# fukangl/SMG-multimodal-grasping

Measured on AMD Instinct MI355X. Metric: affordance fwd+bwd passes/sec (16-rot 224^2 RGB-D), higher is better.
Workload: dtype f32; 1 GPU; 16 rot x 224^2 (S=640): fwd + Huber + bwd + Adam per GPU per step; reinforcement_net style 0; 17 trunk passes; fp32; leg=headline, rotations=16, input_size=640, parallelism=dp1

## Files before the change

### smg-multimodal-grasping_amd/csrc/backward.hip

```cpp
#include "engine.h"

static void pick_chunk(const Plane& pl, int n_planes, int tiles_per_chunk, int& chunk, int& cps, int target = 768) {
    const int want = (target + tiles_per_chunk - 1) / tiles_per_chunk;
    cps = (want + n_planes - 1) / n_planes;
    if (cps < 1) cps = 1;
    chunk = ((pl.HW + cps - 1) / cps + 63) / 64 * 64;
    cps = (pl.HW + chunk - 1) / chunk;
}

int do_backward(smg_engine* e, const smg_net* net, const float* dq, hipStream_t st, int phases) {
    if (!e->have_fwd) return fail(-22, "smg_backward without a preceding smg_forward");
    if (!net->grads) return fail(-22, "net.grads is NULL");
    if (phases == 2 && !e->bw_phase0_done)
        return fail(-22, "smg_backward_phase(1) must follow smg_backward_phase(0) of the same forward");
    if ((phases & 1) && e->bw_phase0_done)
        return fail(-22, "smg_backward / smg_backward_phase(0) while the second half of a two-phase backward is still due (run phase 1 or a new forward)");
    const Layout& L = *e->L;
    const TrunkRef& T = L.trunk[e->f_trunk];
    const HeadRef& Hd = L.head[e->f_head];
    const int NS = e->f_streams, NP = e->f_pairs;
    const float* P = net->params;
    float* Gr = net->grads;
    const Plane p4 = e->p_blk[3];
    const bool ph_a = phases & 1, ph_b = phases & 2;
    if (ph_a) {
        for (int r = 0; r < kStatRep; ++r) HIP_OK(hipMemsetAsync(e->bstat + (size_t)r * kStatRepStride, 0, 2 * e->bstat_span * sizeof(double), st));
    }
    const bool split16 = e->prec == 0 && kSplitOp == 3;
    if (ph_a && split16) HIP_OK(hipMemsetAsync(e->gamax, 0, (size_t)e->gamax_words * sizeof(unsigned), st));
    const hipStream_t s2 = (e->prof || e->serialize) ? st : e->side;
    auto fork = [&](hipEvent_t ev) -> int {
        HIP_OK(hipEventRecord(ev, st));
        HIP_OK(hipStreamWaitEvent(s2, ev, 0));
        return 0;
    };
    const bool gs_materialised = split16 || NS > 4;
    auto gs_on_side = [&](const Plane& pl) { return split16 && !e->generic3x3 && pl.HW <= 1600 && NS <= 4; };
    auto launch_gs_apply = [&](int b, int i, hipStream_t cs, float* GSb) {
        const Plane pl = e->p_blk[b];
        const int Ct = kBlockCtot[b];
        const DenseLayerRef& d = T.layers[b][i];
        BnBwdApplyArgs a{};
        a.g = e->G[b]; a.ldg = Ct; a.gcoff = d.cin; a.x = e->X[b]; a.ldx = Ct; a.xcoff = d.cin; a.pl = pl; a.C = kGrowth;
        a.xsum = fsum(e, e->st_X[b]); a.xsq = fsq(e, e->st_X[b]); a.xstride = Ct; a.xtab = stat_table(e, e->sx_tab[b], e->max_streams, Ct);
        a.s1 = b1(e, e->st_X[b]); a.s2 = b2(e, e->st_X[b]); a.sstride = Ct; a.scoff = d.cin; a.gamma = nullptr; a.eps = kEps;
        a.out = GSb; a.ldo = kGrowth; a.amax = split16 ? gamax_of(e, b, i, 0) : nullptr;
        PREC_DISPATCH(e, launch_kernel(e, bn_bwd_apply_kernel<PREC>, dim3((pl.HWp + bn_apply_rows(PREC) - 1) / bn_apply_rows(PREC), NS), dim3(256), 0, cs,
                                       K_OTHER, 0, ESZ(e) * NS * pl.HW * 3 * kGrowth, false, a));
    };

    if (ph_a) {
    {
        ValueBwdArgs a;
// ... 194 lines not shown
            float* bt = el(e, e->Bt, e->bt_off[b][i]);
            const LayerBuf lb = buf_of(b, i);
            float* GSb = lb.GS;
            float* D2b = lb.D2;
            static_assert(kRing % 3 == 0 && kRing > 3, "the sparse ring wait covers three slots at a time");
            if (lb.ring >= kRing && lb.ring % 3 == 0) HIP_OK(hipStreamWaitEvent(st, e->ev_side[(lb.ring + 2) % kRing], 0));
            GradSrc gsrc{};
            gsrc.g = el(e, e->G[b], d.cin); gsrc.ldg = Ct; gsrc.x = el(e, e->X[b], d.cin); gsrc.ldx = Ct;
            gsrc.xsum = fsum(e, e->st_X[b]) + d.cin; gsrc.xsq = fsq(e, e->st_X[b]) + d.cin;
            gsrc.s1 = b1(e, e->st_X[b]) + d.cin; gsrc.s2 = b2(e, e->st_X[b]) + d.cin; gsrc.sstride = Ct; gsrc.eps = kEps;
            if (e->generic3x3 || (gs_materialised && !gs_on_side(pl))) {
                launch_gs_apply(b, i, st, GSb);
                if (gs_materialised) { gsrc = GradSrc{}; gsrc.g = GSb; gsrc.ldg = kGrowth; gsrc.amax = gamax_of(e, b, i, 0); }
            }
            if (!e->generic3x3) {
                Halo3x3DgradArgs a;
                a.g = gsrc; a.pl = pl; a.C = kBottleneck;
                a.mbuf = bt;
                a.dst = split16 ? e->DY2 : D2b; a.o1 = b1(e, e->st_Bt[b][i]); a.o2 = b2(e, e->st_Bt[b][i]); a.ostride = kBottleneck;
                a.wu = e->packed_u + e->pk_hd[b][i]; a.bt = bn_table(e, e->sb_tab[b][i], e->max_streams, 0, kBottleneck, P + d.n2.w, P + d.n2.b);
                const double flops = 2.0 * NS * pl.HW * 9 * kBottleneck * kGrowth;
                const double bytes = ESZ(e) * NS * pl.HW * (kGrowth + 2 * kBottleneck);
                if (halo_tile(pl, NS) == 16) {
                    a.tiles_x = (pl.W + 15) / 16; a.cg_per_wg = kBottleneck / 32;
                    if (pl.H % 16 || pl.W % 16) {
                        PREC_DISPATCH(e, launch_kernel(e, conv3x3_halo_dgrad_kernel<16, PREC, true>, dim3(((pl.H + 15) / 16) * a.tiles_x, NS), dim3(256),
                                                       HaloDgradSGeo<16, PREC>::smem_bytes(kBottleneck), st, K_D3, flops, bytes, true, a));
                    } else {
                        PREC_DISPATCH(e, launch_kernel(e, conv3x3_halo_dgrad_kernel<16, PREC>, dim3((pl.H / 16) * a.tiles_x, NS), dim3(256),
                                                       HaloDgradSGeo<16, PREC>::smem_bytes(kBottleneck), st, K_D3, flops, bytes, true, a));
                    }
                } else {
                    a.tiles_x = (pl.W + 7) / 8; a.cg_per_wg = 1;
                    PREC_DISPATCH(e, launch_kernel(e, conv3x3_halo_dgrad_kernel<8, PREC>, dim3(((pl.H + 7) / 8) * a.tiles_x, NS, kBottleneck / 64), dim3(256),
                                                   HaloDgradSGeo<8, PREC>::smem_bytes(kBottleneck), st, K_D3, flops, bytes, true, a));
                }
            } else {
                auto run = [&](auto tag) {
                    using Cfg = decltype(tag);
                    BwdDataP<Cfg, true, E_STORE, false> p{};
                    p.gbuf = GSb; p.ldg = kGrowth; p.gcoff = 0; p.xbuf = nullptr; p.pa = pl; p.KA = kGrowth;
                    p.wp = e->packed_u + e->pk_g3d[b][i]; p.K8tot = 9 * kGrowth / 8; p.ldn = kBottleneck; p.wcol0 = 0; p.N = kBottleneck;
                    p.mbuf = bt; p.ldm = kBottleneck; p.mcoff = 0; p.pm = pl;
                    p.msum = fsum(e, e->st_Bt[b][i]); p.msq = fsq(e, e->st_Bt[b][i]); p.mstride = kBottleneck;
                    p.egamma = P + d.n2.w; p.ebeta = P + d.n2.b;
                    p.dst = split16 ? e->DY2 : D2b; p.ldd = kBottleneck; p.dcoff = 0;
                    p.o1 = b1(e, e->st_Bt[b][i]); p.o2 = b2(e, e->st_Bt[b][i]); p.ostride = kBottleneck; p.ocoff = 0;
                    p.dbeta = Gr + d.n2.b; p.dgamma = Gr + d.n2.w; p.eps = kEps;
                    launch_gemm(e, st, p, dim3(NS * pl.HWp / Cfg::BM, kBottleneck / Cfg::BN), K_D3, 2.0 * NS * pl.HW * 9 * kBottleneck * kGrowth,
                                ESZ(e) * NS * pl.HW * (kGrowth + 2 * kBottleneck));
                };
                if (pl.HWp % 128 == 0) run(CfgP128x128{}); else run(CfgP64x128{});
            }
            if (split16) {
                BnBwdApplySplitArgs a{};
                a.g = e->DY2; a.x = bt; a.pl = pl;
                a.xsum = fsum(e, e->st_Bt[b][i]); a.xsq = fsq(e, e->st_Bt[b][i]); a.xstride = kBottleneck; a.xtab = !e->generic3x3 ? stat_table(e, e->sb_tab[b][i], e->max_streams, kBottleneck) : StatTab{};
                a.s1 = b1(e, e->st_Bt[b][i]); a.s2 = b2(e, e->st_Bt[b][i]); a.sstride = kBottleneck;
                a.gamma = P + d.n2.w; a.eps = kEps; a.out = reinterpret_cast<u32x4*>(D2b); a.binv = lb.D2S;
                if (!e->generic3x3) { a.dbeta = Gr + d.n2.b; a.dgamma = Gr + d.n2.w; }
                launch_kernel(e, bn_bwd_apply_split_kernel, dim3(pl.HWp / kScaleBlock, NS), dim3(256), 0, st, K_OTHER, 0, 4.0 * NS * pl.HW * 3 * kBottleneck, false, a);
            } else {
                BnBwdApplyArgs a{};
                a.g = D2b; a.ldg = kBottleneck; a.gcoff = 0; a.x = bt; a.ldx = kBottleneck; a.xcoff = 0; a.pl = pl; a.C = kBottleneck;
                a.xsum = fsum(e, e->st_Bt[b][i]); a.xsq = fsq(e, e->st_Bt[b][i]); a.xstride = kBottleneck; a.xtab = !e->generic3x3 ? stat_table(e, e->sb_tab[b][i], e->max_streams, kBottleneck) : StatTab{};
                a.s1 = b1(e, e->st_Bt[b][i]); a.s2 = b2(e, e->st_Bt[b][i]); a.sstride = kBottleneck; a.scoff = 0;
                a.gamma = P + d.n2.w; a.eps = kEps; a.out = D2b; a.ldo = kBottleneck; a.amax = nullptr;
                if (!e->generic3x3) { a.dbeta = Gr + d.n2.b; a.dgamma = Gr + d.n2.w; }
                PREC_DISPATCH(e, launch_kernel(e, bn_bwd_apply_kernel<PREC>, dim3((pl.HWp + bn_apply_rows(PREC) - 1) / bn_apply_rows(PREC), NS), dim3(256), 0, st,
                                               K_OTHER, 0, ESZ(e) * NS * pl.HW * 3 * kBottleneck, false, a));
            }
            if (fork(e->ev_d2[lb.ring % kRing])) return -5;
            if (int rc = issue_wgrads(b, i)) return rc;
            HIP_OK(hipEventRecord(e->ev_side[lb.ring % kRing], s2));
            if (e->dbg_stop == b * 100 + i && e->prec == 0) {
                const int64_t nf = (int64_t)NS * pl.HWp * Ct;
                if (e->dbg_gsnap_floats < nf) {
                    if (e->dbg_gsnap) (void)hipFree(e->dbg_gsnap);
                    e->dbg_gsnap = nullptr; e->dbg_gsnap_floats = 0;
                    HIP_OK(hipMalloc((void**)&e->dbg_gsnap, (size_t)nf * sizeof(float)));
                    e->dbg_gsnap_floats = nf;
                }
                HIP_OK(hipMemcpyAsync(e->dbg_gsnap, e->G[b], (size_t)nf * sizeof(float), hipMemcpyDeviceToDevice, st));
            }
            const int L = (int)T.layers[b].size();
            const int g_lo = i - ((L - 1 - i) % kGroup == kGroup - 1 ? 0 : std::min(i, kGroup - 1 - (L - 1 - i) % kGroup));
            const int cs = T.layers[b][g_lo].cin;
            if (d.cin > cs) {
                auto run = [&](auto tag, auto ptag) {
                    using Cfg = MC<decltype(tag), decltype(ptag)::value>;
                    BwdDataP<Cfg, false, E_ACCUM, false, decltype(ptag)::value> p{};
                    p.gbuf = D2b; p.ldg = kBottleneck; p.gcoff = 0; p.xbuf = nullptr; p.pa = pl; p.KA = kBottleneck; p.binv = lb.D2S;
                    p.wp = e->packed_u + e->pk_d1[b][i]; p.K8tot = kBottleneck / 8; p.ldn = d.cin; p.wcol0 = cs; p.N = d.cin - cs;
                    p.mbuf = e->X[b]; p.ldm = Ct; p.mcoff = cs; p.pm = pl;
                    p.msum = fsum(e, e->st_X[b]); p.msq = fsq(e, e->st_X[b]); p.mstride = Ct; p.mtab = stat_table(e, e->sx_tab[b], e->max_streams, Ct);
                    p.egamma = P + d.n1.w + cs; p.ebeta = P + d.n1.b + cs;
                    p.dst = e->G[b]; p.ldd = Ct; p.dcoff = cs;
                    p.o1 = b1(e, e->st_X[b]); p.o2 = b2(e, e->st_X[b]); p.ostride = Ct; p.ocoff = cs;
                    p.dbeta = e->dbscr + e->db_off[b][i] + cs; p.dgamma = e->dbscr + e->db_off[b][i] + d.cin + cs; p.rep_stride = e->db_total; p.eps = kEps;
                    launch_gemm(e, st, p, dim3(NS * pl.HWp / Cfg::BM, (p.N + Cfg::BN - 1) / Cfg::BN), K_D1, 2.0 * NS * pl.HW * p.N * kBottleneck,
                                ESZ(e) * NS * pl.HW * (kBottleneck + 3.0 * p.N));
                };
                PREC_DISPATCH(e, if (pl.HWp % 128 == 0) run(CfgP128x64{}, PTAG); else run(CfgP64x64{}, PTAG));
            }
            if (i == g_lo) {
                auto run = [&](auto tag, auto ptag) {
                    using Cfg = MC<decltype(tag), decltype(ptag)::value>;
                    BwdDataGroupP<Cfg, decltype(ptag)::value> p{};
                    const int g_hi = L - 1 - ((L - 1 - g_lo) / kGroup) * kGroup;
                    p.nseg = g_hi - g_lo + 1;
                    for (int k = 0; k < p.nseg; ++k) {
                        const DenseLayerRef& dk = T.layers[b][g_lo + k];
                        const LayerBuf lk = buf_of(b, g_lo + k);
                        p.seg[k].g = lk.D2; p.seg[k].wp = e->packed_u + e->pk_d1[b][g_lo + k]; p.seg[k].ldn = dk.cin; p.seg[k].binv = lk.D2S;
                        p.seg[k].gamma = P + dk.n1.w; p.seg[k].beta = P + dk.n1.b;
                        p.seg[k].dbeta = e->dbscr + e->db_off[b][g_lo + k]; p.seg[k].dgamma = e->dbscr + e->db_off[b][g_lo + k] + dk.cin;
                    }
                    p.ldg = kBottleneck; p.pa = pl; p.KA = kBottleneck; p.N = cs;
                    p.mbuf = e->X[b]; p.ldm = Ct;
                    p.msum = fsum(e, e->st_X[b]); p.msq = fsq(e, e->st_X[b]); p.mstride = Ct; p.mtab = stat_table(e, e->sx_tab[b], e->max_streams, Ct);
                    p.dst = e->G[b]; p.ldd = Ct;
                    p.o1 = b1(e, e->st_X[b]); p.o2 = b2(e, e->st_X[b]); p.ostride = Ct; p.rep_stride = e->db_total; p.eps = kEps;
                    launch_gemm(e, st, p, dim3(NS * pl.HWp / Cfg::BM, (cs + Cfg::BN - 1) / Cfg::BN), K_D1, 2.0 * NS * pl.HW * cs * kBottleneck * p.nseg,
                                ESZ(e) * NS * pl.HW * ((double)p.nseg * kBottleneck + 3.0 * cs));
                };
                PREC_DISPATCH(e, if (pl.HWp % 128 == 0) run(GemmCfg<128, 64, 32, 2, 2, 1, true>{}, PTAG); else run(CfgP64x64{}, PTAG));
            }
            if (e->dbg_stop == b * 100 + i) return debug_stop();
        }
        if (b > 0) {
            const Plane pp = e->p_blk[b - 1];
            const int Cp = kBlockCtot[b - 1], C0 = kBlockCin[b];
            {
                int chunk, cps;
                pick_chunk(pl, NS, (C0 / 128) * (Cp / 128), chunk, cps);
                auto go = [&](auto ptag) -> int {
                BwdWeightP<MC<CfgW128x128, decltype(ptag)::value>, W_POOL, C_IDENT, 1, true, decltype(ptag)::value> p{};
                p.gbuf = e->G[b]; p.ldg = Ct; p.gcoff = 0; p.xbuf = e->X[b]; p.ldx = Ct; p.xcoff = 0; p.pa = pl; p.MA = C0;
                p.xsum = fsum(e, e->st_X[b]); p.xsq = fsq(e, e->st_X[b]); p.xstride = Ct;
                p.s1 = b1(e, e->st_X[b]); p.s2 = b2(e, e->st_X[b]); p.sstride = Ct; p.scoff = 0; p.agamma = nullptr;
                p.bbuf = e->X[b - 1]; p.ldb = Cp; p.pb = pp; p.NB = Cp;
// ... 93 lines not shown
```

### smg-multimodal-grasping_amd/csrc/engine.h

```cpp
#pragma once
#include <hip/hip_runtime.h>

#include <algorithm>
#include <cmath>
#include <cstdio>
#include <cstdlib>
#include <cstring>
#include <string>
#include <type_traits>
#include <vector>

#include "../../include/smg_hip.h"
#include "elem.cuh"
#include "gemm.cuh"
#include "halo.cuh"
#include "ws.cuh"
#include "wsw.cuh"
#include "plan.h"

using namespace smg;

int smg_fail(int code, const std::string& msg);
static inline int fail(int code, const std::string& msg) { return smg_fail(code, msg); }
#define HIP_OK(expr)                                                                              \
// ... 34 lines not shown

constexpr int kGroup = GROUP_MAX;
constexpr int kRing = kGroup + 2;

constexpr int kDbRep = 8;
struct DbSeg { int64_t grad_off; int scr_off; int n; };

struct ProfRec { hipEvent_t a, b; int kind; double flops; int stage; double bytes; };

struct StatArr { int64_t off; int stride; };

struct smg_engine {
    int device = 0, S = 0, max_streams = 0, max_pairs = 0, head_out = 1;
    Plane p_img, p_stem, p_blk[4];
    int OH = 1, OW = 1;
    const Layout* L = nullptr;

    float* img4 = nullptr; float* stem = nullptr; float* X[4] = {}; float* Bt = nullptr;
    std::vector<int64_t> bt_off[4];
    unsigned char* argmax = nullptr;
    float* F = nullptr; float* H1 = nullptr;
    float* G[4] = {}; float* GS[kRing] = {}; float* D2[kRing] = {}; float* part = nullptr; int64_t part_floats = 0;
    float* DY2 = nullptr; float* D2S[kRing] = {};
    hipStream_t side = nullptr; hipEvent_t ev_gs[kRing] = {}, ev_d2[kRing] = {}, ev_side[kRing] = {}, ev_misc = nullptr, ev_end = nullptr; float* DY0 = nullptr; float* DH1 = nullptr; float* DF = nullptr;
    double* fstat = nullptr; int64_t fstat_span = 0;
    double* bstat = nullptr; int64_t bstat_span = 0;
    float* dbscr = nullptr; int db_total = 0; int db_off[4][24] = {}; int db_toff[3] = {}; struct DbSeg* d_dbseg = nullptr; int n_dbseg = 0;
    StatArr st_stem, st_X[4], st_F, st_H1; std::vector<StatArr> st_Bt[4];
    u32x4* packed_u = nullptr; int64_t packed_units = 0;
    float* packed_f = nullptr; int64_t packed_floats = 0;
    PackDesc* d_pack = nullptr; std::vector<PackDesc> h_pack[3]; std::vector<PackDesc> h_pack_head[3];
    int pack_stride = 0, bnupd_stride = 0, n_bnupd = 0;
    int64_t pk_conv0 = 0, pk_conv0_1 = 0, pk_head0 = 0, pk_hd0 = 0, pk_head1 = 0;
    std::vector<int64_t> pk_c1[4], pk_d1[4], pk_g3f[4], pk_g3d[4], pk_hf[4], pk_hd[4]; int64_t pk_t[3] = {}, pk_td[3] = {};
    int max_pack = 0;
    float* asc = nullptr; ActScaleDesc* d_asc = nullptr; int n_asc = 0;
    unsigned* gamax = nullptr; int64_t gamax_words = 0;
    float* stab = nullptr; int64_t stab_floats = 0;
    int64_t sx_tab[4] = {}, sb_tab[4][24] = {}, sf_tab = 0;
    BnUpdDesc* d_bnupd = nullptr;
    bool have_fwd = false; int f_trunk = 0, f_head = 0, f_streams = 0, f_pairs = 0;
    bool bw_phase0_done = false;
    bool f_stem1 = false;
    int* d_stream_image = nullptr; int* d_stream_rot = nullptr; int* d_pair_a = nullptr; int* d_pair_b = nullptr;
    int* d_seq_t = nullptr; int* d_seq_h = nullptr; int* d_user_ptr = nullptr; int* d_user_pair = nullptr; int* d_user_slot = nullptr;
    float* d_affine = nullptr;
    int* d_stage = nullptr; int* h_stage[2] = {}; hipEvent_t ev_stage[2] = {}; int stage_ints = 0, stage_turn = 0;
    int so_image = 0, so_rot = 0, so_pa = 0, so_pb = 0, so_seq_t = 0, so_seq_h = 0, so_uptr = 0, so_upair = 0, so_uslot = 0, so_aff = 0, so_ma = 0, so_mb = 0, so_adam = 0;
    bool capturing = false; int* h_stage_g = nullptr; hipEvent_t ev_graph = nullptr, ev_gin = nullptr; hipStream_t gstream = nullptr; struct StepGraph* step_graph = nullptr;
    int64_t workspace_bytes = 0;
    int n_cu = 256;
    int prec = 0;
    bool serialize = false;
    bool deterministic = false;
    bool generic3x3 = false, generic_c1 = false, generic_w1 = false;
    int dbg_stop = -1;
    float* dbg_gsnap = nullptr; int64_t dbg_gsnap_floats = 0;
    bool prof = false; std::vector<ProfRec> recs; std::vector<hipEvent_t> ev_pool;
    double prof_ms[5][K_COUNT] = {}; int64_t prof_n[5][K_COUNT] = {}; double prof_flops[5][K_COUNT] = {}; double prof_bytes[5][K_COUNT] = {}; int prof_stage = -1;
    int launch_rc = 0;
};

static inline int halo_tile(const Plane& p, int n_streams = 1 << 20) {
    return (int64_t)((p.H + 15) / 16) * ((p.W + 15) / 16) * n_streams >= 200 ? 16 : 8;
}

static int w3_tiles_per_wg(int n_tiles, int ts, int n_streams, int64_t part_floats, double fix_scale = 1.0) {
    const double fix = (ts == 16 ? 0.6 : 2.4) * fix_scale;
    double best = 1e30;
    int tpw_best = 1;
    for (int tpw = 1; tpw <= n_tiles; ++tpw) {
        const int g = (n_tiles + tpw - 1) / tpw;
        const int rounds = (g * (kBottleneck / 32) * n_streams + 511) / 512;
        const double cost = rounds * (tpw + fix);
        if (cost < best - 1e-9) { best = cost; tpw_best = tpw; }
    }
    while (tpw_best < n_tiles && (int64_t)((n_tiles + tpw_best - 1) / tpw_best) * n_streams * 9 * 32 * kBottleneck > part_floats) ++tpw_best;
    return tpw_best;
}

static Plane make_plane(int H, int W) {
    Plane p; p.H = H; p.W = W; p.HW = H * W;
    const int g = p.HW >= 8192 ? 128 : 64;
    p.HWp = (p.HW + g - 1) / g * g;
    return p;
}

template <class T>
static int dev_alloc(smg_engine* e, T** out, int64_t count) {
    void* p = nullptr;
    hipError_t err = hipMalloc(&p, (size_t)count * sizeof(T));
    if (err != hipSuccess) return fail(-12, std::string("hipMalloc ") + std::to_string(count * sizeof(T)) + " B: " + hipGetErrorString(err));
    e->workspace_bytes += count * (int64_t)sizeof(T);
    *out = (T*)p;
    return 0;
}
#define ALLOC(ptr, count) do { int _r = dev_alloc(e, &(ptr), (count)); if (_r) return _r; } while (0)

static hipEvent_t prof_event(smg_engine* e) {
    if (!e->ev_pool.empty()) { hipEvent_t ev = e->ev_pool.back(); e->ev_pool.pop_back(); return ev; }
    hipEvent_t ev; (void)hipEventCreate(&ev); return ev;
}
#define ESZ(e) ((e)->prec ? 2.0 : 4.0)
struct ProfScope {
    smg_engine* e; hipStream_t st; int kind; double flops, bytes; hipEvent_t a{}, b{};
    ProfScope(smg_engine* e_, hipStream_t s, int k, double f, double by) : e(e_), st(s), kind(k), flops(f), bytes(by) {
// ... 183 lines not shown
```

### smg-multimodal-grasping_amd/csrc/engine.hip

```cpp
#include "engine.h"

static thread_local std::string g_err;
int smg_fail(int code, const std::string& msg) { g_err = msg; return code; }

static int engine_build(smg_engine* e) {
    const Layout& L = *e->L;
    const int NS = e->max_streams, NP = e->max_pairs;
    const int S = e->S;
    const int H1 = (S - 1) / 2 + 1, H2 = (H1 - 1) / 2 + 1;
    e->p_img = make_plane(S, S);
    e->p_stem = make_plane(H1, H1);
    int h = H2;
    for (int b = 0; b < 4; ++b) { e->p_blk[b] = make_plane(h, h); h /= 2; }
    e->OH = e->OW = e->p_blk[3].H - kHeadKernel + 1;
    if (e->OH < 1) return fail(-22, "input_size too small for the 20x20 value head");

    if (getenv("SMG_SERIALIZE")) e->serialize = true;
    const int cross = getenv("SMG_CROSSCHECK") ? atoi(getenv("SMG_CROSSCHECK")) : 0;
    e->generic3x3 = cross & 1; e->generic_c1 = cross & 2; e->generic_w1 = cross & 4;

    ALLOC(e->img4, (int64_t)NS * e->p_img.HWp * 4);
    ALLOC(e->stem, (int64_t)NS * e->p_stem.HWp * 64);
    ALLOC(e->DY0, (int64_t)NS * e->p_stem.HWp * 64);
    ALLOC(e->argmax, (int64_t)NS * e->p_blk[0].HWp * 64);
// ... 439 lines not shown
    float* sc = reinterpret_cast<float*>(e->h_stage_g + e->so_adam);
    adam_scalars(adam, adam->step_trunk, sc);
    adam_scalars(adam, adam->step_head, sc + 2);
    HIP_OK(hipEventRecord(e->ev_gin, caller));
    HIP_OK(hipStreamWaitEvent(st, e->ev_gin, 0));
    e->capturing = true;
    int rc = 0;
    if (!g->warm) {
        rc = step_body(e, net, trunk_id, head_id, B, loss_mode, labels_dev, q_out_dev, loss_out_dev, dq_dev, adam, st);
        g->warm = rc == 0;
    } else {
        if (!g->exec) {
            hipError_t err = hipStreamBeginCapture(st, hipStreamCaptureModeRelaxed);
            if (err != hipSuccess) { e->capturing = false; return fail(-5, std::string("hipStreamBeginCapture: ") + hipGetErrorString(err)); }
            rc = step_body(e, net, trunk_id, head_id, B, loss_mode, labels_dev, q_out_dev, loss_out_dev, dq_dev, adam, st);
            err = hipStreamEndCapture(st, &g->graph);
            if (rc == 0 && err != hipSuccess) rc = fail(-5, std::string("hipStreamEndCapture: ") + hipGetErrorString(err));
            if (rc == 0) {
                err = hipGraphInstantiate(&g->exec, g->graph, nullptr, nullptr, 0);
                if (err != hipSuccess) rc = fail(-5, std::string("hipGraphInstantiate: ") + hipGetErrorString(err));
            }
            if (rc) { e->capturing = false; step_graph_drop(e); return rc; }
        }
        hipError_t err = hipGraphLaunch(g->exec, st);
        if (err != hipSuccess) rc = fail(-5, std::string("hipGraphLaunch: ") + hipGetErrorString(err));
        e->have_fwd = true; e->bw_phase0_done = false; e->f_trunk = trunk_id; e->f_head = head_id; e->f_streams = B->n_streams; e->f_pairs = B->n_pairs;
        e->f_stem1 = B->heightmaps_dev != nullptr;
    }
    e->capturing = false;
    if (rc == 0) {
        HIP_OK(hipEventRecord(e->ev_graph, st));
        HIP_OK(hipStreamWaitEvent(caller, e->ev_graph, 0));
    }
    return rc;
}

int smg_engine_set_precision(smg_engine* e, int precision) {
    if (!e) return fail(-22, "engine is NULL");
    if (precision < 0 || precision > 2) return fail(-22, "precision must be 0 (fp32 storage, fp32-class split products), 1 (bf16 storage) or 2 (fp16 activations, bf16 gradients)");
    if (precision && e->generic3x3) return fail(-22, "SMG_CROSSCHECK=1 (the generic implicit-GEMM 3x3 path) exists in the fp32-class mode only");
    e->prec = precision;
    step_graph_drop(e);
    e->have_fwd = false;
    e->bw_phase0_done = false;
    return 0;
}

int smg_engine_set_option(smg_engine* e, const char* name, int value) {
    if (!e || !name) return fail(-22, "NULL argument");
    const std::string s(name);
    if (s == "deterministic") { e->deterministic = value != 0; return 0; }
    if (s == "serialize") { e->serialize = value != 0; return 0; }
    if (s == "debug_stop") { e->dbg_stop = value; return 0; }
    return fail(-22, "unknown engine option '" + s + "'");
}

int smg_heightmap(const double* depth_img_dev, int h, int w, const double* intrinsics3x3, const double* cam_pose4x4,
                  const double* inv_homography3x3, int out_w, int out_h, double* out_dev, void* stream) {
    if (!depth_img_dev || !intrinsics3x3 || !cam_pose4x4 || !inv_homography3x3 || !out_dev || h < 1 || w < 1 || out_w < 1 || out_h < 1)
        return fail(-22, "bad heightmap arguments");
    hipPointerAttribute_t attr;
    HIP_OK(hipPointerGetAttributes(&attr, depth_img_dev));
    HIP_OK(hipSetDevice(attr.device));
    HeightmapArgs a;
    a.depth = depth_img_dev; a.h = h; a.w = w;
    a.fx = intrinsics3x3[0]; a.fy = intrinsics3x3[4]; a.cx = intrinsics3x3[2]; a.cy = intrinsics3x3[5];
    a.r20 = cam_pose4x4[8]; a.r21 = cam_pose4x4[9]; a.r22 = cam_pose4x4[10]; a.t2 = cam_pose4x4[11];
    for (int i = 0; i < 9; ++i) a.mi[i] = inv_homography3x3[i];
    a.out = out_dev; a.ow = out_w; a.oh = out_h;
    hipLaunchKernelGGL(heightmap_warp_kernel, dim3((out_w + 255) / 256, out_h), dim3(256), 0, (hipStream_t)stream, a);
    HIP_OK(hipGetLastError());
    return 0;
}

int smg_argmax(const float* values_dev, int n, int* idx_out_dev, float* val_out_dev, void* stream) {
    if (!values_dev || !idx_out_dev || !val_out_dev || n < 1) return fail(-22, "bad argmax arguments");
    hipPointerAttribute_t attr;
    HIP_OK(hipPointerGetAttributes(&attr, values_dev));
    HIP_OK(hipSetDevice(attr.device));
    hipLaunchKernelGGL(argmax_kernel, dim3(1), dim3(256), 0, (hipStream_t)stream, values_dev, n, idx_out_dev, val_out_dev);
    HIP_OK(hipGetLastError());
    return 0;
}

int smg_adam_step(float* params, const float* grads, float* m, float* v, int64_t offset, int64_t count, int step, float lr,
                  float beta1, float beta2, float eps, void* stream) {
    if (!params || !grads || !m || !v || count < 0 || step < 1) return fail(-22, "bad Adam arguments");
    const double bc1 = 1.0 - std::pow((double)beta1, step), bc2 = 1.0 - std::pow((double)beta2, step);
    const float step_size = (float)((double)lr / bc1);
    const float bc2_sqrt = (float)std::sqrt(bc2);
    if (count == 0) return 0;
    {
        hipPointerAttribute_t attr;
        HIP_OK(hipPointerGetAttributes(&attr, params));
        HIP_OK(hipSetDevice(attr.device));
    }
    int blocks = (int)((count + 255) / 256);
    if (blocks > 4096) blocks = 4096;
    hipLaunchKernelGGL(adam_kernel, dim3(blocks), dim3(256), 0, (hipStream_t)stream, params + offset, grads + offset, m + offset, v + offset,
                       count, step_size, beta1, beta2, eps, 1.0f, bc2_sqrt);
    HIP_OK(hipGetLastError());
    return 0;
}

int64_t smg_debug_read(smg_engine* e, const char* name, float* host_out, int64_t cap, void* stream) {
    if (!e || !name) return fail(-22, "NULL argument");
    const int NS = e->max_streams, NP = e->max_pairs;
    const float* src = nullptr; int64_t n = 0;
    std::string s(name);
    if (s == "img") {
        src = e->img4; n = (int64_t)NS * e->p_img.HWp * 4;
        if (e->f_stem1 && host_out) {
            if (cap < n) return fail(-22, "img: buffer too small");
            HIP_OK(hipSetDevice(e->device));
            HIP_OK(hipStreamSynchronize((hipStream_t)stream));
            std::vector<float> one((size_t)(n / 4));
            HIP_OK(hipMemcpy(one.data(), src, one.size() * sizeof(float), hipMemcpyDeviceToHost));
            for (int64_t i = 0; i < n / 4; ++i) { host_out[4 * i] = host_out[4 * i + 1] = host_out[4 * i + 2] = one[(size_t)i]; host_out[4 * i + 3] = 0.f; }
            return n;
        }
    }
    else if (s == "stem") { src = e->stem; n = (int64_t)NS * e->p_stem.HWp * 64; }
    else if (s == "dy0") { src = e->DY0; n = (int64_t)NS * e->p_stem.HWp * 64; }
    else if (s == "feat") { src = e->F; n = (int64_t)NP * e->p_blk[3].HWp * 2 * kFeat; }
    else if (s == "h1") { src = e->H1; n = (int64_t)NP * e->p_blk[3].HWp * kHeadMid; }
    else if (s == "df") { src = e->DF; n = (int64_t)NP * e->p_blk[3].HWp * 2 * kFeat; }
    else if (s == "dh1") { src = e->DH1; n = (int64_t)NP * e->p_blk[3].HWp * kHeadMid; }
    else if (s.size() == 2 && (s[0] == 'x' || s[0] == 'g') && s[1] >= '1' && s[1] <= '4') {
        const int b = s[1] - '1';
        src = s[0] == 'x' ? e->X[b] : e->G[b]; n = (int64_t)NS * e->p_blk[b].HWp * kBlockCtot[b];
    } else if (s.size() >= 4 && s.substr(0, 2) == "bt") {
        int b = 0, i = 0;
        if (std::sscanf(name, "bt%d_%d", &b, &i) != 2 || b < 1 || b > 4 || i < 1 || i > kBlockLayers[b - 1]) return fail(-22, "bad bt name");
        src = el(e, e->Bt, e->bt_off[b - 1][i - 1]); n = (int64_t)NS * e->p_blk[b - 1].HWp * kBottleneck;
    } else if (s == "gsnap") {
        src = e->dbg_gsnap; n = e->dbg_gsnap_floats;
        if (!src) return fail(-22, "gsnap: no debug_stop backward has run");
    } else if (s == "dy2") {
        src = e->DY2; n = (int64_t)NS * e->p_blk[0].HWp * kBottleneck;
    } else if (s.size() >= 5 && (s.substr(0, 3) == "gs_" || s.substr(0, 3) == "d2_")) {
        int b = 0, i = 0;
        if (std::sscanf(name + 3, "%d_%d", &b, &i) != 2 || b < 1 || b > 4 || i < 1 || i > kBlockLayers[b - 1]) return fail(-22, "bad ring buffer name");
        const int slot = ring_pos(b - 1, i - 1) % kRing;
        const Plane& pl = e->p_blk[b - 1];
        const bool gs = s[0] == 'g';
        const int64_t per_stream = (int64_t)pl.HWp * (gs ? kGrowth : kBottleneck);
        n = (int64_t)NS * per_stream;
        if (!host_out) return n;
        const int ns_out = (int)std::min<int64_t>(NS, cap / per_stream);
        n = ns_out * per_stream;
        if (e->prec != 0) return fail(-22, "ring buffer debug reads exist in precision mode 0 only");
        HIP_OK(hipSetDevice(e->device));
        HIP_OK(hipStreamSynchronize((hipStream_t)stream));
        if (gs || kSplitOp != 3) {
            HIP_OK(hipMemcpy(host_out, gs ? e->GS[slot] : e->D2[slot], n * sizeof(float), hipMemcpyDeviceToHost));
            return n;
        }
        std::vector<unsigned short> u((size_t)ns_out * per_stream * 2);
        std::vector<float> inv((size_t)NS * (pl.HWp / kScaleBlock));
        HIP_OK(hipMemcpy(u.data(), e->D2[slot], u.size() * sizeof(unsigned short), hipMemcpyDeviceToHost));
        HIP_OK(hipMemcpy(inv.data(), e->D2S[slot], inv.size() * sizeof(float), hipMemcpyDeviceToHost));
        auto h2f = [](unsigned h) -> double {
            const int ex = (h >> 10) & 31, man = h & 1023;
            const double v = ex == 0 ? std::ldexp((double)man, -24) : (ex == 31 ? (man ? NAN : INFINITY) : std::ldexp((double)(man | 1024), ex - 25));
            return (h & 0x8000u) ? -v : v;
        };
        for (int sn = 0; sn < ns_out; ++sn)
            for (int k8 = 0; k8 < kD2K8; ++k8)
                for (int p = 0; p < pl.HWp; ++p) {
                    const size_t uh = ((((size_t)sn * 2 + 0) * kD2K8 + k8) * pl.HWp + p) * 8, ul = ((((size_t)sn * 2 + 1) * kD2K8 + k8) * pl.HWp + p) * 8;
                    const double iv = inv[(size_t)sn * (pl.HWp / kScaleBlock) + p / kScaleBlock];
                    for (int j = 0; j < 8; ++j)
                        host_out[((size_t)sn * pl.HWp + p) * kBottleneck + 8 * k8 + j] = (float)((h2f(u[uh + j]) + h2f(u[ul + j])) * iv);
                }
        return n;
    } else if (s == "asc") {
        src = e->asc; n = 2 * e->n_asc;
    } else if (s.size() >= 6 && s.substr(0, 5) == "fs_bt") {
        int b = 0, i = 0;
        if (std::sscanf(name, "fs_bt%d_%d", &b, &i) != 2 || b < 1 || b > 4 || i < 1 || i > kBlockLayers[b - 1]) return fail(-22, "bad fs_bt name");
        n = (int64_t)4 * NS * kBottleneck;
        if (!host_out) return n;
        if (cap < n) return fail(-22, "fs_bt: buffer too small");
        HIP_OK(hipSetDevice(e->device));
        HIP_OK(hipStreamSynchronize((hipStream_t)stream));
        HIP_OK(hipMemcpy(host_out, fsum(e, e->st_Bt[b - 1][i - 1]), (size_t)NS * kBottleneck * sizeof(double), hipMemcpyDeviceToHost));
        HIP_OK(hipMemcpy(host_out + 2 * NS * kBottleneck, fsq(e, e->st_Bt[b - 1][i - 1]), (size_t)NS * kBottleneck * sizeof(double), hipMemcpyDeviceToHost));
        return n;
    } else return fail(-22, "unknown debug buffer");
    if (!host_out) return n;
    if (cap < n) n = cap;
    HIP_OK(hipSetDevice(e->device));
// ... 69 lines not shown
```

Baseline: 64.29 passes/s.

## Fuse split BN-backward apply with narrow 1x1 data-gradient GEMM

Result: no change. 63.85 passes/s (median of 2 runs) (-0.7%).

```diff
diff --git a/smg-multimodal-grasping_amd/csrc/backward.hip b/smg-multimodal-grasping_amd/csrc/backward.hip
--- a/smg-multimodal-grasping_amd/csrc/backward.hip
+++ b/smg-multimodal-grasping_amd/csrc/backward.hip
@@ -1,4 +1,5 @@
 #include "engine.h"
+#include "fused_d1.cuh"
 
 static void pick_chunk(const Plane& pl, int n_planes, int tiles_per_chunk, int& chunk, int& cps, int target = 768) {
     const int want = (target + tiles_per_chunk - 1) / tiles_per_chunk;
@@ -299,6 +300,20 @@
                 };
                 if (pl.HWp % 128 == 0) run(CfgP128x128{}); else run(CfgP64x128{});
             }
+            const int L = (int)T.layers[b].size();
+            const int g_lo = i - ((L - 1 - i) % kGroup == kGroup - 1 ? 0 : std::min(i, kGroup - 1 - (L - 1 - i) % kGroup));
+            const int cs = T.layers[b][g_lo].cin;
+            const bool fused = split16 && !e->generic3x3 && e->fuse_d1 && d.cin > cs;
+            if (e->dbg_stop == b * 100 + i && e->prec == 0) {
+                const int64_t nf = (int64_t)NS * pl.HWp * Ct;
+                if (e->dbg_gsnap_floats < nf) {
+                    if (e->dbg_gsnap) (void)hipFree(e->dbg_gsnap);
+                    e->dbg_gsnap = nullptr; e->dbg_gsnap_floats = 0;
+                    HIP_OK(hipMalloc((void**)&e->dbg_gsnap, (size_t)nf * sizeof(float)));
+                    e->dbg_gsnap_floats = nf;
+                }
+                HIP_OK(hipMemcpyAsync(e->dbg_gsnap, e->G[b], (size_t)nf * sizeof(float), hipMemcpyDeviceToDevice, st));
+            }
             if (split16) {
                 BnBwdApplySplitArgs a{};
                 a.g = e->DY2; a.x = bt; a.pl = pl;
@@ -306,6 +321,27 @@
                 a.s1 = b1(e, e->st_Bt[b][i]); a.s2 = b2(e, e->st_Bt[b][i]); a.sstride = kBottleneck;
                 a.gamma = P + d.n2.w; a.eps = kEps; a.out = reinterpret_cast<u32x4*>(D2b); a.binv = lb.D2S;
                 if (!e->generic3x3) { a.dbeta = Gr + d.n2.b; a.dgamma = Gr + d.n2.w; }
+                if (fused) {
+                    auto run = [&](auto tag) {
+                        using Cfg = decltype(tag);
+                        FusedD1Args<Cfg> fa{};
+                        fa.a = a;
+                        auto& p = fa.p;
+                        p.gbuf = nullptr; p.xbuf = nullptr; p.pa = pl; p.KA = kBottleneck; p.binv = nullptr;
+                        p.wp = e->packed_u + e->pk_d1[b][i]; p.K8tot = kBottleneck / 8; p.ldn = d.cin; p.wcol0 = cs; p.N = d.cin - cs;
+                        p.mbuf = e->X[b]; p.ldm = Ct; p.mcoff = cs; p.pm = pl;
+                        p.msum = fsum(e, e->st_X[b]); p.msq = fsq(e, e->st_X[b]); p.mstride = Ct; p.mtab = stat_table(e, e->sx_tab[b], e->max_streams, Ct);
+                        p.egamma = P + d.n1.w + cs; p.ebeta = P + d.n1.b + cs;
+                        p.dst = e->G[b]; p.ldd = Ct; p.dcoff = cs;
+                        p.o1 = b1(e, e->st_X[b]); p.o2 = b2(e, e->st_X[b]); p.ostride = Ct; p.ocoff = cs;
+                        p.dbeta = e->dbscr + e->db_off[b][i] + cs; p.dgamma = e->dbscr + e->db_off[b][i] + d.cin + cs; p.rep_stride = e->db_total; p.eps = kEps;
+                        p.tm = TileMap{0, 0, 0};
+                        launch_kernel(e, bn_bwd_apply_d1_fused_kernel<Cfg>, dim3(pl.HWp / kScaleBlock, NS), dim3(256), FusedD1Geo<Cfg>::SMEM_BYTES, st, K_D1,
+                                      2.0 * NS * pl.HW * p.N * kBottleneck, 4.0 * NS * pl.HW * 3 * kBottleneck + 4.0 * NS * pl.HW * 3.0 * p.N, false, fa);
+                    };
+                    if (d.cin - cs > 96 || (d.cin - cs) % 32) return fail(-22, "fused 1x1 data gradient: a layer group's narrow range is 32, 64 or 96 columns");
+                    if (d.cin - cs > 64) run(CfgFused128{}); else run(CfgFused64{});
+                } else
                 launch_kernel(e, bn_bwd_apply_split_kernel, dim3(pl.HWp / kScaleBlock, NS), dim3(256), 0, st, K_OTHER, 0, 4.0 * NS * pl.HW * 3 * kBottleneck, false, a);
             } else {
                 BnBwdApplyArgs a{};
@@ -320,20 +356,7 @@
             if (fork(e->ev_d2[lb.ring % kRing])) return -5;
             if (int rc = issue_wgrads(b, i)) return rc;
             HIP_OK(hipEventRecord(e->ev_side[lb.ring % kRing], s2));
-            if (e->dbg_stop == b * 100 + i && e->prec == 0) {
-                const int64_t nf = (int64_t)NS * pl.HWp * Ct;
-                if (e->dbg_gsnap_floats < nf) {
-                    if (e->dbg_gsnap) (void)hipFree(e->dbg_gsnap);
-                    e->dbg_gsnap = nullptr; e->dbg_gsnap_floats = 0;
-                    HIP_OK(hipMalloc((void**)&e->dbg_gsnap, (size_t)nf * sizeof(float)));
-                    e->dbg_gsnap_floats = nf;
-                }
-                HIP_OK(hipMemcpyAsync(e->dbg_gsnap, e->G[b], (size_t)nf * sizeof(float), hipMemcpyDeviceToDevice, st));
-            }
-            const int L = (int)T.layers[b].size();
-            const int g_lo = i - ((L - 1 - i) % kGroup == kGroup - 1 ? 0 : std::min(i, kGroup - 1 - (L - 1 - i) % kGroup));
-            const int cs = T.layers[b][g_lo].cin;
-            if (d.cin > cs) {
+            if (d.cin > cs && !fused) {
                 auto run = [&](auto tag, auto ptag) {
                     using Cfg = MC<decltype(tag), decltype(ptag)::value>;
                     BwdDataP<Cfg, false, E_ACCUM, false, decltype(ptag)::value> p{};
diff --git a/smg-multimodal-grasping_amd/csrc/engine.h b/smg-multimodal-grasping_amd/csrc/engine.h
--- a/smg-multimodal-grasping_amd/csrc/engine.h
+++ b/smg-multimodal-grasping_amd/csrc/engine.h
@@ -110,6 +110,7 @@
     int n_cu = 256;
     int prec = 0;
     bool serialize = false;
+    bool fuse_d1 = true;
     bool deterministic = false;
     bool generic3x3 = false, generic_c1 = false, generic_w1 = false;
     int dbg_stop = -1;
diff --git a/smg-multimodal-grasping_amd/csrc/engine.hip b/smg-multimodal-grasping_amd/csrc/engine.hip
--- a/smg-multimodal-grasping_amd/csrc/engine.hip
+++ b/smg-multimodal-grasping_amd/csrc/engine.hip
@@ -515,6 +515,7 @@
     if (s == "deterministic") { e->deterministic = value != 0; return 0; }
     if (s == "serialize") { e->serialize = value != 0; return 0; }
     if (s == "debug_stop") { e->dbg_stop = value; return 0; }
+    if (s == "fuse_d1") { e->fuse_d1 = value != 0; step_graph_drop(e); return 0; }
     return fail(-22, "unknown engine option '" + s + "'");
 }
 
@@ -601,6 +602,14 @@
         if (!src) return fail(-22, "gsnap: no debug_stop backward has run");
     } else if (s == "dy2") {
         src = e->DY2; n = (int64_t)NS * e->p_blk[0].HWp * kBottleneck;
+    } else if (s.size() >= 6 && (s.substr(0, 4) == "d2u_" || s.substr(0, 4) == "d2s_")) {
+        int b = 0, i = 0;
+        if (std::sscanf(name + 4, "%d_%d", &b, &i) != 2 || b < 1 || b > 4 || i < 1 || i > kBlockLayers[b - 1]) return fail(-22, "bad ring buffer name");
+        if (e->prec != 0) return fail(-22, "ring buffer debug reads exist in precision mode 0 only");
+        const int slot = ring_pos(b - 1, i - 1) % kRing;
+        const Plane& pl = e->p_blk[b - 1];
+        if (s[2] == 'u') { src = e->D2[slot]; n = (int64_t)NS * pl.HWp * kBottleneck; }
+        else { src = e->D2S[slot]; n = (int64_t)NS * (pl.HWp / kScaleBlock); }
     } else if (s.size() >= 5 && (s.substr(0, 3) == "gs_" || s.substr(0, 3) == "d2_")) {
         int b = 0, i = 0;
         if (std::sscanf(name + 3, "%d_%d", &b, &i) != 2 || b < 1 || b > 4 || i < 1 || i > kBlockLayers[b - 1]) return fail(-22, "bad ring buffer name");
diff --git a/smg-multimodal-grasping_amd/csrc/fused_d1.cuh b/smg-multimodal-grasping_amd/csrc/fused_d1.cuh
--- /dev/null
+++ b/smg-multimodal-grasping_amd/csrc/fused_d1.cuh
@@ -0,0 +1,179 @@
+#pragma once
+#include "elem.cuh"
+#include "gemm.cuh"
+
+namespace smg {
+
+using CfgFused64 = GemmCfg<64, 64, 16, 2, 2, 1, true>;
+using CfgFused128 = GemmCfg<64, 128, 16, 2, 2, 1, true>;
+template <class Cfg> using FusedD1Policy = BwdDataP<Cfg, false, E_ACCUM, false, 0>;
+
+template <class Cfg>
+struct FusedD1Geo {
+    static constexpr int LDA = Cfg::BN > 64 ? kScaleBlock : kScaleBlock + 4;
+    static constexpr int NST = 3;
+    static constexpr int A_BYTES = 2 * kD2K8 * LDA * 16;
+    static constexpr int DPT = Cfg::BN > 64 ? 2 : 1;
+    static constexpr int B_STAGE_UNITS = Cfg::BN > 64 ? 4 * 96 : 4 * 64;
+    static constexpr int B_BYTES = NST * B_STAGE_UNITS * 16;
+    static constexpr int PARAM_FLOATS = 5 * Cfg::BN;
+    static_assert(B_STAGE_UNITS * 16 >= 4 * 8 * kD2K8 * 4, "the apply's parameters fit a weight stage");
+    static constexpr int SMEM_BYTES = A_BYTES + B_BYTES + PARAM_FLOATS * 4;
+    static_assert(B_BYTES >= 2 * Cfg::WM * Cfg::BN * 4, "the epilogue's column reduction reuses the weight stages");
+};
+
+template <class Cfg>
+struct FusedD1Args {
+    BnBwdApplySplitArgs a;
+    FusedD1Policy<Cfg> p;
+};
+
+template <class Cfg>
+static __global__ __launch_bounds__(256, 3) void bn_bwd_apply_d1_fused_kernel(const FusedD1Args<Cfg> fa) {
+    using Z = FusedD1Geo<Cfg>;
+    using P = FusedD1Policy<Cfg>;
+    static_assert(Cfg::BM == kScaleBlock && Cfg::TM == 1 && Cfg::WM == 2 && Cfg::WN == 2, "one scale block per workgroup, one 32-row tile per wave");
+    static_assert(P::kOp == 3 && P::kAUnit, "the fp16-split unit form");
+    constexpr int C = 8 * kD2K8;
+    extern __shared__ __attribute__((aligned(16))) float smem[];
+    __shared__ float red[4];
+    char* As = reinterpret_cast<char*>(smem);
+    char* Bs = As + Z::A_BYTES;
+    float* prm = reinterpret_cast<float*>(Bs + (Z::NST - 1) * Z::B_STAGE_UNITS * 16);
+    float* sp = reinterpret_cast<float*>(Bs + Z::B_BYTES) - 4 * C;
+    const BnBwdApplySplitArgs& a = fa.a;
+    const P& p = fa.p;
+
+    const int n = blockIdx.y, t = threadIdx.x, lane = t & 63, wave = t >> 6;
+    const int l31 = lane & 31, half = lane >> 5;
+    const int wm0 = (wave / Cfg::WN) * 32, wn0 = (wave % Cfg::WN) * Cfg::TN * 32;
+    const int cs = t >> 3, rr = t & 7;
+    const int pbase = blockIdx.x * kScaleBlock;
+    const int r0 = pbase + rr;
+    const bool product = pbase < a.pl.HW;
+    const int N = p.N;
+
+    float4 gv[8], xv[8];
+#pragma unroll
+    for (int k = 0; k < 8; ++k) {
+        const int r = r0 + 8 * k;
+        const int64_t pix = (int64_t)n * a.pl.HWp + (r < a.pl.HW ? r : 0);
+        gv[k] = ld4(a.g + pix * C + 4 * cs);
+        xv[k] = ld4(a.x + pix * C + 4 * cs);
+    }
+    const unsigned lds0 = (unsigned)(uintptr_t)As;
+    const int n_runs = 4 * N / 64;
+    unsigned b_voff[Z::DPT], b_dst[Z::DPT];
+#pragma unroll
+    for (int i = 0; i < Z::DPT; ++i) {
+        const int run = min(wave + 4 * i, n_runs - 1);
+        const int id = run * 64 + lane, q = id / N, r = id - q * N;
+        b_voff[i] = 16u * (unsigned)(((q >> 1) * p.K8tot + (q & 1)) * p.ldn + r);
+        b_dst[i] = lds0 + (unsigned)Z::A_BYTES + 16u * (unsigned)(run * 64);
+    }
+    auto dma_tile = [&](int kt, int st) {
+#pragma unroll
+        for (int i = 0; i < Z::DPT; ++i)
+            dma_unit(UnitSrc{p.wp, kWholeBuf, b_voff[i], 16u * (unsigned)(kt * 2 * p.ldn + p.wcol0)}, b_dst[i] + (unsigned)(st * Z::B_STAGE_UNITS * 16));
+    };
+    if (product) { dma_tile(0, 0); dma_tile(1, 1); }
+
+    if (t < C) {
+        const double inv = 1.0 / (double)a.pl.HW;
+        float mean, invstd;
+        tab_or_moments(a.xtab, n, t, a.xsum, a.xsq, (int64_t)n * a.xstride + t, inv, a.eps, mean, invstd);
+        const double s1 = stat_get(a.s1, (int64_t)n * a.sstride + t), s2 = stat_get(a.s2, (int64_t)n * a.sstride + t);
+        prm[t] = a.gamma[t] * invstd;
+        prm[C + t] = (float)(s1 * inv);
+        prm[2 * C + t] = mean;
+        prm[3 * C + t] = invstd * (float)(s2 * inv);
+        if (a.dbeta && blockIdx.x == 0) {
+            atomicAdd(a.dbeta + t, (float)s1);
+            atomicAdd(a.dgamma + t, (float)s2);
+        }
+    }
+    typename P::Ctx ctx;
+    ctx.n = n; ctx.n0 = 0;
+    ctx.m0 = sgpr(n * a.pl.HWp + pbase);
+    ctx.whole = P::kEarly && pbase + Cfg::BM <= a.pl.HW && (Cfg::BN <= N || (N & 31) == 0);
+    if (product) p.init_params(ctx, sp);
+    __syncthreads();
+    float vmax = 0.f;
+#pragma unroll
+    for (int k = 0; k < 8; ++k) {
+        const float4 o = r0 + 8 * k < a.pl.HW ? affine2(gv[k], xv[k], prm + 4 * cs, C) : zero4();
+        gv[k] = o;
+        vmax = fmaxf(fmaxf(vmax, fmaxf(fabsf(o.x), fabsf(o.y))), fmaxf(fabsf(o.z), fabsf(o.w)));
+    }
+    __builtin_amdgcn_sched_barrier(0);
+    if (product) p.early_fetch(ctx);
+#pragma unroll
+    for (int o = 32; o > 0; o >>= 1) vmax = fmaxf(vmax, __shfl_xor(vmax, o));
+    if ((t & 63) == 0) red[t >> 6] = vmax;
+    __syncthreads();
+    vmax = fmaxf(fmaxf(red[0], red[1]), fmaxf(red[2], red[3]));
+    ActScale sc{1.f, 1.f};
+    if (vmax > 0.f) sc = scale_of_max(__float_as_uint(vmax));
+    if (t == 0) a.binv[(int64_t)n * (a.pl.HWp / kScaleBlock) + blockIdx.x] = sc.inv;
+    ctx.ginv[0] = ctx.ginv[1] = sc.inv * pack_inv_scale(p.wp);
+#pragma unroll
+    for (int k = 0; k < 8; ++k) {
+        const Split4 s = split4<3>(mul4(gv[k], sc.s));
+        char* at = As + (((cs >> 1) * Z::LDA + rr + 8 * k) * 16 + (cs & 1) * 8);
+        *reinterpret_cast<uint2*>(at) = s.p[0];
+        *reinterpret_cast<uint2*>(at + kD2K8 * Z::LDA * 16) = s.p[1];
+    }
+    auto store_units = [&]() {
+        u32x4* ob = a.out + d2_stream_units(n, a.pl.HWp) + pbase;
+#pragma unroll
+        for (int i = 0; i < 2 * kD2K8 * kScaleBlock / 256; ++i) {
+            const int id = t + 256 * i, plane = id / kScaleBlock, row = id % kScaleBlock;
+            ob[(int64_t)plane * a.pl.HWp + row] = *reinterpret_cast<const u32x4*>(As + (plane * Z::LDA + row) * 16);
+        }
+    };
+    if (!product) {
+        __syncthreads();
+        store_units();
+        return;
+    }
+
+    f32x16 acc[Cfg::TM][Cfg::TN];
+#pragma unroll
+    for (int j = 0; j < Cfg::TN; ++j)
+#pragma unroll
+        for (int r = 0; r < 16; ++r) acc[0][j][r] = 0.f;
+    bool jok[Cfg::TN];
+#pragma unroll
+    for (int j = 0; j < Cfg::TN; ++j) jok[j] = wn0 + j * 32 + 32 <= N;
+    auto compute = [&](int kt, int st) {
+        const char* A = As + ((kt * 2 + half) * Z::LDA + wm0 + l31) * 16;
+        const char* B = Bs + st * Z::B_STAGE_UNITS * 16 + (half * N + wn0 + l31) * 16;
+        const u32x4 ah = *reinterpret_cast<const u32x4*>(A), al = *reinterpret_cast<const u32x4*>(A + kD2K8 * Z::LDA * 16);
+        u32x4 bh[Cfg::TN], bl[Cfg::TN];
+#pragma unroll
+        for (int j = 0; j < Cfg::TN; ++j) {
+            bh[j] = bl[j] = u32x4{0u, 0u, 0u, 0u};
+            if (jok[j]) {
+                bh[j] = *reinterpret_cast<const u32x4*>(B + j * 32 * 16);
+                bl[j] = *reinterpret_cast<const u32x4*>(B + (2 * N + j * 32) * 16);
+            }
+        }
+#pragma unroll
+        for (int g = 0; g < 3; ++g)
+#pragma unroll
+            for (int j = 0; j < Cfg::TN; ++j)
+                if (jok[j]) acc[0][j] = mfma_f16(g == 1 ? al : ah, g == 0 ? bl[j] : bh[j], acc[0][j]);
+    };
+    constexpr int KT = kD2K8 / 2;
+#pragma unroll
+    for (int kt = 0; kt < KT; ++kt) {
+        if (kt == 0 || kt + 1 == KT) dma_wait<0>(); else dma_wait<Z::DPT>();
+        dma_barrier();
+        if (kt + 2 < KT) dma_tile(kt + 2, (kt + 2) % Z::NST);
+        compute(kt, kt % Z::NST);
+    }
+    store_units();
+    p.epilogue(ctx, acc, reinterpret_cast<float*>(Bs), sp, true);
+}
+
+}
```
